# yinyunie/Pose2Room

Hardware: AMD Instinct MI355X
Metric: P2RNet train-step samples/sec (T=1024,J=53,bs=32) (higher is better)
Workload: dtype f32; 1 GPU; P2RNet full train step, bs=32/GPU, T=1024, J=53, seeds=512, proposals=128 (BASELINE configs[2]); input=P2RNet_dataloader over SyntheticPoseDataset, global_batch=32, frames=1024, parallelism=dp1

## Files before the change

### pose2room_amd/csrc/stgcn_gcn3_dcoef_body.h

```cpp
#include "gcn3_sched.inc"

#ifndef D3_MARK
#define D3_TRACE_TILE(tile)
#define D3_MARK(i)
#endif
namespace {

constexpr int D3_F = TILE_F, D3_NW = TILE_NW, D3_SLOTS = TILE_SLOTS, D3_V = TILE_V;
constexpr int D3_RS = TILE_RS, D3_BUF = TILE_BUF, D3_NV4 = TILE_NV4, D3_PW = TILE_PW;
static_assert(G3_V == TILE_V, "schedule generated for another skeleton");

struct D3Common {
  int T, ltot;
  int tiles_per_seq, total_tiles;
};
struct D3Params : D3Common, D3Extra {};

constexpr int d3_slot_joints[D3_NW][D3_SLOTS] = G3_SLOT_JOINTS_1;
constexpr int d3_plane0[D3_NW] = G3_PLANE0_1;

template <int NE, int O0, int O1, int O2, int O3, int O4, int O5>
__device__ __forceinline__ void d3_gather(const char *xl, float (&dv)[6][4]) {
  constexpr int off[6] = {O0, O1, O2, O3, O4, O5};
#pragma unroll
  for (int j = 0; j < NE; ++j)
#pragma unroll
    for (int q = 0; q < 4; ++q) dv[j][q] = *reinterpret_cast<const float *>(xl + off[j] + q * 4 * D3_RS * 4);
}

template <int CTRL>
__device__ __forceinline__ float d3_add_dpp(float v) {
  return v + __int_as_float(__builtin_amdgcn_update_dpp(0, __float_as_int(v), CTRL, 0xf, 0xf, true));
}
template <int OFF>
__device__ __forceinline__ void d3_lane_add(unsigned base, float v, unsigned long long mask) {
  asm volatile("s_mov_b64 exec, %2\n\tds_add_f32 %0, %1 offset:%3\n\ts_mov_b64 exec, -1"
               : : "v"(base), "v"(v), "s"(mask), "n"(OFF) : "memory");
}
template <int NE, int C0, int C1, int C2, int C3, int C4, int C5>
__device__ __forceinline__ void d3_reduce(const f32x4 &h, const float (&dv)[6][4], unsigned dcs) {
  constexpr unsigned long long L31 = 1ull << 31, L63 = 1ull << 63;
  constexpr int NP = NE / 2, NV = NP + (NE & 1);
  const f32x2 h01 = {h[0], h[1]}, h23 = {h[2], h[3]};
  float t[NE];
#pragma unroll
  for (int j = 0; j < NE; ++j) {
    f32x2 pr = h01 * f32x2{dv[j][0], dv[j][1]};
    pr = __builtin_elementwise_fma(h23, f32x2{dv[j][2], dv[j][3]}, pr);
    t[j] = pr.x + pr.y;
  }
  float v[NV];
#pragma unroll
  for (int q = 0; q < NP; ++q) {
    auto sw = __builtin_amdgcn_permlane32_swap(__float_as_uint(t[2 * q]), __float_as_uint(t[2 * q + 1]), false, false);
    v[q] = __uint_as_float(sw[0]) + __uint_as_float(sw[1]);
  }
  if (NE & 1) v[NP] = t[NE - 1];
#pragma unroll
  for (int q = 0; q < NV; ++q) v[q] = d3_add_dpp<0xB1>(v[q]);
#pragma unroll
  for (int q = 0; q < NV; ++q) v[q] = d3_add_dpp<0x4E>(v[q]);
#pragma unroll
  for (int q = 0; q < NV; ++q) v[q] = d3_add_dpp<0x141>(v[q]);
#pragma unroll
  for (int q = 0; q < NV; ++q) v[q] = d3_add_dpp<0x140>(v[q]);
#pragma unroll
  for (int q = 0; q < NV; ++q) v[q] = d3_add_dpp<0x142>(v[q]);
  if (NE & 1) v[NP] = d3_add_dpp<0x143>(v[NP]);
  if (NP > 0) { d3_lane_add<4 * C0>(dcs, v[0], L31); d3_lane_add<4 * C1>(dcs, v[0], L63); }
  if (NP > 1) { d3_lane_add<4 * C2>(dcs, v[1], L31); d3_lane_add<4 * C3>(dcs, v[1], L63); }
  if (NP > 2) { d3_lane_add<4 * C4>(dcs, v[2], L31); d3_lane_add<4 * C5>(dcs, v[2], L63); }
  if (NE == 1) d3_lane_add<4 * C0>(dcs, v[0], L63);
  if (NE == 3) d3_lane_add<4 * C2>(dcs, v[1], L63);
  if (NE == 5) d3_lane_add<4 * C4>(dcs, v[2], L63);
}

#define D3_VISIT(set, plane, next, wrap, piece)                                      \
  {                                                                                  \
    load_a(aS[(set) ^ 1], next, (wrap) ? ((ph + 1) & 3) : ph);                        \
    if ((piece) >= 0 && copy) dma_piece(piece);                                      \
  }
#define D3_STEP(set, slot, ne, o0, c0, o1, c1, o2, c2, o3, c3, o4, c4, o5, c5)   \
  {                                                                              \
    float dv_[6][4];                                                             \
    d3_gather<ne, o0, o1, o2, o3, o4, o5>(xl, dv_);                              \
    if (D3_FENCED) __builtin_amdgcn_sched_barrier(0);                            \
    d3_product(h, aS[set], bz[slot]);                                            \
    if (D3_FENCED) __builtin_amdgcn_sched_barrier(0);                            \
    d3_reduce<ne, c0, c1, c2, c3, c4, c5>(h, dv_, dcs_off);                      \
  }
#define D3_CONT(ne, o0, c0, o1, c1, o2, c2, o3, c3, o4, c4, o5, c5)   \
  {                                                                   \
    float dv_[6][4];                                                  \
    d3_gather<ne, o0, o1, o2, o3, o4, o5>(xl, dv_);                   \
    d3_reduce<ne, c0, c1, c2, c3, c4, c5>(h, dv_, dcs_off);           \
  }
#define D3_END(parity, pieces)                                                            \
  {                                                                                       \
    if (copy) { _Pragma("unroll") for (int i_ = pieces; i_ < D3_PW; ++i_) dma_piece(i_); } \
    if (parity) d3_copy_a(aS[0], aS[1]);                                                  \
  }

template <int WAVE>
__device__ __forceinline__ void d3_wave_main(const D3Params &p, float *lds, const float *__restrict__ x,
                                             const float *__restrict__ dz, const D3W *__restrict__ W, float xscale) {
  constexpr int V = D3_V, RS = D3_RS, BUF = D3_BUF, NW = D3_NW, SLOTS = D3_SLOTS;
  constexpr int wave = WAVE;
  unsigned dcs_off = (unsigned)(2 * BUF * sizeof(float));
  asm volatile("" : "+v"(dcs_off));
  const int tid = threadIdx.x;
  const int lane = tid & 63;
  const int g = lane >> 4, r = lane & 15;
  constexpr const int (&sj)[SLOTS] = d3_slot_joints[WAVE];

  const size_t row_stride = (size_t)p.T * V;
  const char *xl0 = reinterpret_cast<const char *>(lds + g * RS + r * V);

  int doff[D3_PW];
#pragma unroll
  for (int i = 0; i < D3_PW; ++i) {
    const int pc = i * NW + wave;
    const int e = pc * 64 + lane;
    const int lrow = e / (RS / 4), c4 = e - lrow * (RS / 4);
    const int row = 4 * (lrow & 3) + (lrow >> 2);
    doff[i] = (pc < TILE_PIECES && e < D3_NV4) ? (int)(((size_t)row * row_stride + 4 * c4) * sizeof(float)) : -1;
  }
  D3B bz[SLOTS];
  D3A aS[2];
  f32x4 h;
  auto load_a = [&](D3A &a, int k, int ph) { d3_load_a(a, W, k, ph, lane); };

  int tile = blockIdx.x;
  if (tile < p.total_tiles) {
    const int seq = tile / p.tiles_per_seq, t0 = (tile % p.tiles_per_seq) * D3_F;
    const float *dr = dz + (size_t)seq * 64 * row_stride + (size_t)t0 * V;
#pragma unroll
    for (int i = 0; i < D3_PW; ++i)
      if (doff[i] >= 0) tile_dma16(dr, doff[i], lds + (i * NW + wave) * 256);
  }
  load_a(aS[0], d3_plane0[WAVE], 0);

  for (; tile < p.total_tiles; tile += gridDim.x) {
    const int seq = tile / p.tiles_per_seq, t0 = (tile % p.tiles_per_seq) * D3_F;
    const float *dg = dz + (size_t)seq * 64 * row_stride + (size_t)t0 * V;
    const int ntile = tile + gridDim.x;
    const bool has_next = ntile < p.total_tiles;
    const int nseq = has_next ? ntile / p.tiles_per_seq : 0, nt0 = has_next ? (ntile % p.tiles_per_seq) * D3_F : 0;
    const float *ndg = dz + (size_t)nseq * 64 * row_stride + (size_t)nt0 * V;
    D3_TRACE_TILE(tile);
    D3_MARK(0);

    {
      float *xb = lds + BUF;
      const char *xr = reinterpret_cast<const char *>(xb + 4 * g * RS + r * V);
      const float *xs = x + (size_t)seq * 64 * row_stride + (size_t)t0 * V;
#pragma unroll
      for (int sl = 0; sl < 4; ++sl) {
        asm volatile("s_waitcnt lgkmcnt(0)" ::: "memory");
        __syncthreads();
#pragma unroll
        for (int i = 0; i < D3_PW; ++i)
          if (doff[i] >= 0) tile_dma16(xs + (size_t)sl * 16 * row_stride, doff[i], xb + (i * NW + wave) * 256);
        asm volatile("s_waitcnt vmcnt(0)" ::: "memory");
        __syncthreads();
#pragma unroll
        for (int i = 0; i < SLOTS; ++i)
          if (sj[i] >= 0) d3_read_x(bz[i], xr, sj[i], sl, xscale);
      }
      asm volatile("s_waitcnt lgkmcnt(0)" ::: "memory");
    }

#pragma unroll 1
    for (int ph = 0; ph < 4; ++ph) {
      D3_MARK(1 + 3 * ph);
      asm volatile("s_waitcnt vmcnt(0)" ::: "memory");
      D3_MARK(2 + 3 * ph);
      __syncthreads();
      D3_MARK(3 + 3 * ph);
      float *buf_nxt = lds + ((ph + 1) & 1) * BUF;
      const char *xl = xl0 + (ph & 1) * BUF * sizeof(float);
      const bool copy = ph + 1 < 4 || has_next;
      const float *src = (ph + 1 < 4) ? dg + (size_t)(ph + 1) * 16 * row_stride : ndg;
      auto dma_piece = [&](int i) {
        if (doff[i] >= 0) tile_dma16(src, doff[i], buf_nxt + (i * NW + wave) * 256);
      };
      if constexpr (WAVE == 0) { D3_BODY_0 } else if constexpr (WAVE == 1) { D3_BODY_1 }
      else if constexpr (WAVE == 2) { D3_BODY_2 } else if constexpr (WAVE == 3) { D3_BODY_3 }
      else if constexpr (WAVE == 4) { D3_BODY_4 } else if constexpr (WAVE == 5) { D3_BODY_5 }
      else if constexpr (WAVE == 6) { D3_BODY_6 } else { D3_BODY_7 }
    }
    D3_MARK(13);
  }
}

__global__ __launch_bounds__(D3_NW * 64, 2) void D3_KERNEL(D3Params p, const float *__restrict__ x,
                                                           const float *__restrict__ dz, const D3W *__restrict__ W,
                                                           float *__restrict__ dcoef_partial) {
  extern __shared__ float lds[];
  float *dcs = lds + 2 * D3_BUF;
  const int tid = threadIdx.x;
  for (int e = tid; e < p.ltot * D3_V; e += D3_NW * 64) dcs[e] = 0.f;
  float xscale, inv;
  d3_scales(p, xscale, inv);
  __syncthreads();
  switch (__builtin_amdgcn_readfirstlane(tid >> 6)) {
    case 0: d3_wave_main<0>(p, lds, x, dz, W, xscale); break;
    case 1: d3_wave_main<1>(p, lds, x, dz, W, xscale); break;
    case 2: d3_wave_main<2>(p, lds, x, dz, W, xscale); break;
    case 3: d3_wave_main<3>(p, lds, x, dz, W, xscale); break;
    case 4: d3_wave_main<4>(p, lds, x, dz, W, xscale); break;
    case 5: d3_wave_main<5>(p, lds, x, dz, W, xscale); break;
    case 6: d3_wave_main<6>(p, lds, x, dz, W, xscale); break;
    default: d3_wave_main<7>(p, lds, x, dz, W, xscale); break;
  }
  __syncthreads();
  float *out = dcoef_partial + (size_t)blockIdx.x * p.ltot * D3_V;
  for (int e = tid; e < p.ltot * D3_V; e += D3_NW * 64) out[e] = dcs[e] * inv;
}

int d3_launch(int N, int T, int V, int K, int ltot, const float *x, const float *dz, const D3W *W, int n_blocks,
              float *dcoef_partial, void *stream, const D3Extra &extra) {
  if (N < 0 || T <= 0 || V != D3_V || K != G3_K || ltot <= 0 || n_blocks < 1) return P2R_EINVAL;
  if (T % D3_F != 0 || ((uintptr_t)dz % 16) != 0) return P2R_EINVAL;
  if (N == 0) return hipMemsetAsync(dcoef_partial, 0, (size_t)n_blocks * ltot * V * sizeof(float), p2r_stream(stream));
  D3Params p;
  static_cast<D3Extra &>(p) = extra;
  p.T = T; p.ltot = ltot;
  p.tiles_per_seq = T / D3_F;
  const long long tiles = (long long)N * p.tiles_per_seq;
  if (tiles > 0x7fffffffLL) return P2R_EINVAL;
  p.total_tiles = (int)tiles;
  const size_t lds = (size_t)2 * D3_BUF * sizeof(float) + (size_t)ltot * V * sizeof(float);
  if (lds > 160 * 1024) return P2R_EINVAL;
  return p2r_launch_big_lds<D3_KERNEL>(n_blocks, D3_NW * 64, lds, stream, p, x, dz, W, dcoef_partial);
}

}
```

### pose2room_amd/csrc/stgcn_gcn3_dw.hip

```cpp
#include "stgcn_tile.h"

#include "gcn3_sched.inc"

namespace {

constexpr int W3_F = 4;
constexpr int W3_V = TILE_V;
constexpr int W3_NW = TILE_NW;
constexpr int W3_RL = W3_F * W3_V;
constexpr int W3_TILE = 64 * W3_RL;
constexpr int W3_NV4 = W3_TILE / 4;
constexpr int W3_PW = tile_pw(W3_NV4);
static_assert(G3_V == TILE_V, "schedule generated for another skeleton");
constexpr int W3_CS = (64 * W3_V + W3_NW * 64 - 1) / (W3_NW * 64);

struct W3Params {
  int T, ltot;
  int tiles_per_seq, total_tiles;
};

constexpr int w3_wave_set[W3_NW] = W3_WAVE_SET;
constexpr int w3_wave_half[W3_NW] = W3_WAVE_HALF;
constexpr int w3_set_planes[4][W3_MAXPL] = W3_SET_PLANES;

__device__ __forceinline__ void w3_mfma8(f32x4 (&acc)[2][4], const float (&a)[4], const f32x2 &b) {
  asm volatile(
      "s_nop 1\n\t"
      "v_mfma_f32_16x16x4_f32 %0, %8, %12, %0\n\tv_mfma_f32_16x16x4_f32 %1, %9, %12, %1\n\t"
      "v_mfma_f32_16x16x4_f32 %2, %10, %12, %2\n\tv_mfma_f32_16x16x4_f32 %3, %11, %12, %3\n\t"
      "v_mfma_f32_16x16x4_f32 %4, %8, %13, %4\n\tv_mfma_f32_16x16x4_f32 %5, %9, %13, %5\n\t"
      "v_mfma_f32_16x16x4_f32 %6, %10, %13, %6\n\tv_mfma_f32_16x16x4_f32 %7, %11, %13, %7"
      : "+v"(acc[0][0]), "+v"(acc[0][1]), "+v"(acc[0][2]), "+v"(acc[0][3]), "+v"(acc[1][0]), "+v"(acc[1][1]),
        "+v"(acc[1][2]), "+v"(acc[1][3])
      : "v"(a[0]), "v"(a[1]), "v"(a[2]), "v"(a[3]), "v"(b.x), "v"(b.y));
}

constexpr int W3_MAXNE = 12;

template <int NE>
__device__ __forceinline__ void w3_gather_n(const char *dl, const char *cl, const int (&off)[W3_MAXNE],
                                            const int (&ci)[W3_MAXNE], f32x2 (&dv)[W3_MAXNE], float (&cf)[W3_MAXNE]) {
#pragma unroll
  for (int j = 0; j < NE; ++j) {
    dv[j].x = *reinterpret_cast<const float *>(dl + off[j]);
    dv[j].y = *reinterpret_cast<const float *>(dl + off[j] + 16 * W3_RL * 4);
    cf[j] = *reinterpret_cast<const float *>(cl + 4 * ci[j]);
  }
}
template <int NE>
__device__ __forceinline__ f32x2 w3_combine(const f32x2 (&dv)[W3_MAXNE], const float (&cf)[W3_MAXNE]) {
  f32x2 v = dv[0] * f32x2{cf[0], cf[0]};
#pragma unroll
  for (int j = 1; j < NE; ++j) v = __builtin_elementwise_fma(dv[j], f32x2{cf[j], cf[j]}, v);
  return v;
}

#define W3_UNPACK(o0, c0, o1, c1, o2, c2, o3, c3, o4, c4, o5, c5, o6, c6, o7, c7, o8, c8, o9, c9, o10, c10, o11, c11) \
  constexpr int off_[W3_MAXNE] = {o0, o1, o2, o3, o4, o5, o6, o7, o8, o9, o10, o11};                                   \
  constexpr int ci_[W3_MAXNE] = {c0, c1, c2, c3, c4, c5, c6, c7, c8, c9, c10, c11};

#define W3_A(set, joint)                                                                            \
  {                                                                                                 \
    _Pragma("unroll") for (int m_ = 0; m_ < 4; ++m_)                                                \
        aS[set][m_] = *reinterpret_cast<const float *>(xl + 4 * (joint) + m_ * 16 * W3_RL * 4);      \
  }
#define W3_FIRST(ne, ...)                                        \
  {                                                              \
    W3_UNPACK(__VA_ARGS__)                                       \
    f32x2 dv_[W3_MAXNE]; float cf_[W3_MAXNE];                    \
    w3_gather_n<ne>(dl, cl, off_, ci_, dv_, cf_);                \
    b_cur = w3_combine<ne>(dv_, cf_);                            \
  }
#define W3_STEP(aset, slot, ne, ...)                             \
  {                                                              \
    W3_UNPACK(__VA_ARGS__)                                       \
    f32x2 dv_[W3_MAXNE]; float cf_[W3_MAXNE];                    \
    w3_gather_n<ne>(dl, cl, off_, ci_, dv_, cf_);                \
    __builtin_amdgcn_sched_barrier(0);                           \
    w3_mfma8(acc[slot], aS[aset], b_cur);                        \
    __builtin_amdgcn_sched_barrier(0);                           \
    b_cur = w3_combine<ne>(dv_, cf_);                            \
  }
#define W3_LAST(aset, slot)                \
  {                                        \
    __builtin_amdgcn_sched_barrier(0);     \
    w3_mfma8(acc[slot], aS[aset], b_cur);  \
  }

template <int WAVE>
__device__ __forceinline__ void w3_wave_main(const W3Params &p, float *lds, const float *__restrict__ x,
                                             const float *__restrict__ dz, float *__restrict__ dw_partial,
                                             float *__restrict__ colsum_partial) {
  constexpr int V = W3_V, RL = W3_RL, NW = W3_NW;
  constexpr int SET = w3_wave_set[WAVE], HALF = w3_wave_half[WAVE];
  constexpr int wave = WAVE;
  float *xs = lds;
  float *ds = lds + W3_TILE;
  float *coef_l = lds + 2 * W3_TILE;
  const int tid = threadIdx.x;
  const int lane = tid & 63;
  const int g = lane >> 4, r = lane & 15;
  const size_t row_stride = (size_t)p.T * V;

  const char *xl = reinterpret_cast<const char *>(xs + r * RL + g * V);
  const char *dl = reinterpret_cast<const char *>(ds + (32 * HALF + r) * RL + g * V);
  unsigned cl_off = (unsigned)((coef_l - lds) * sizeof(float));
  asm volatile("" : "+v"(cl_off));
  const char *cl = reinterpret_cast<const char *>(lds) + cl_off;

  unsigned doff[W3_PW];
#pragma unroll
  for (int i = 0; i < W3_PW; ++i) {
    const int pc = i * NW + wave, e = pc * 64 + lane;
    const int row = e / (RL / 4), c4 = e - row * (RL / 4);
    doff[i] = (pc < tile_pieces(W3_NV4) && e < W3_NV4) ? (unsigned)(((size_t)row * row_stride + 4 * c4) * sizeof(float)) : 0xffffffffu;
  }
  auto copy_tile = [&](int tile) {
    const int seq = tile / p.tiles_per_seq, t0 = (tile % p.tiles_per_seq) * W3_F;
    const float *xg = x + (size_t)seq * 64 * row_stride + (size_t)t0 * V;
    const float *dg = dz + (size_t)seq * 64 * row_stride + (size_t)t0 * V;
#pragma unroll
    for (int i = 0; i < W3_PW; ++i)
      if (doff[i] != 0xffffffffu) {
        tile_dma16(xg, doff[i], xs + (i * NW + wave) * 256);
        tile_dma16(dg, doff[i], ds + (i * NW + wave) * 256);
      }
  };

  f32x4 acc[W3_MAXPL][2][4];
#pragma unroll
  for (int s = 0; s < W3_MAXPL; ++s)
#pragma unroll
    for (int n = 0; n < 2; ++n)
#pragma unroll
      for (int m = 0; m < 4; ++m) acc[s][n][m] = f32x4{0.f, 0.f, 0.f, 0.f};
  float aS[2][4];
  f32x2 b_cur;
  float cs[W3_CS];
  int cso[W3_CS];
#pragma unroll
  for (int i = 0; i < W3_CS; ++i) {
    cs[i] = 0.f;
    const int idx = tid + NW * 64 * i;
    cso[i] = idx < 64 * V ? (idx / V) * RL + idx % V : 0;
  }

  const int per_xcd = (gridDim.x & 7) == 0 ? (int)(gridDim.x >> 3) : 0;
  const int xcd = blockIdx.x & 7, slot = blockIdx.x >> 3;
  auto tile_of = [&](int i) { return per_xcd ? (i * 8 + xcd) * per_xcd + slot : (int)(blockIdx.x + i * gridDim.x); };
  int it = 0;
  int tile = tile_of(0);
  for (int d = 0; d < (int)((per_xcd ? slot : blockIdx.x) & 3); ++d) __builtin_amdgcn_s_sleep(127);
  if (tile < p.total_tiles) copy_tile(tile);
  for (; tile < p.total_tiles; tile = tile_of(++it)) {
    asm volatile("s_waitcnt vmcnt(0)" ::: "memory");
    __syncthreads();

    if (colsum_partial) {
      float dv4[W3_CS][4];
#pragma unroll
      for (int i = 0; i < W3_CS; ++i)
#pragma unroll
        for (int f = 0; f < 4; ++f) dv4[i][f] = ds[cso[i] + f * V];
#pragma unroll
      for (int i = 0; i < W3_CS; ++i) cs[i] += (dv4[i][0] + dv4[i][1]) + (dv4[i][2] + dv4[i][3]);
    }
    if constexpr (SET == 0) { W3_BODY_0 } else if constexpr (SET == 1) { W3_BODY_1 }
    else if constexpr (SET == 2) { W3_BODY_2 } else { W3_BODY_3 }

    __syncthreads();
    const int ntile = tile_of(it + 1);
    if (ntile < p.total_tiles) copy_tile(ntile);
  }

  if (colsum_partial) {
#pragma unroll
    for (int i = 0; i < W3_CS; ++i) {
      const int idx = tid + NW * 64 * i;
      if (idx < 64 * V) colsum_partial[(size_t)blockIdx.x * 64 * V + idx] = cs[i];
    }
  }
  float *out = dw_partial + (size_t)blockIdx.x * G3_K * 64 * 64;
#pragma unroll
  for (int s = 0; s < W3_MAXPL; ++s) {
    const int k = w3_set_planes[SET][s];
    if (k < 0) continue;
#pragma unroll
    for (int n = 0; n < 2; ++n)
#pragma unroll
      for (int m = 0; m < 4; ++m)
#pragma unroll
        for (int q = 0; q < 4; ++q)
          out[((size_t)k * 64 + 16 * m + 4 * g + q) * 64 + 32 * HALF + 16 * n + r] = acc[s][n][m][q];
  }
}

__global__ __launch_bounds__(W3_NW * 64, 2) void gcn3_dw_kernel(W3Params p, const float *__restrict__ x,
                                                                const float *__restrict__ dz,
                                                                const float *__restrict__ coef,
                                                                float *__restrict__ dw_partial,
                                                                float *__restrict__ colsum_partial) {
  extern __shared__ float lds[];
  float *coef_l = lds + 2 * W3_TILE;
  const int tid = threadIdx.x;
  for (int e = tid; e < p.ltot * W3_V; e += W3_NW * 64) coef_l[e] = coef[e];
  __syncthreads();
  switch (__builtin_amdgcn_readfirstlane(tid >> 6)) {
    case 0: w3_wave_main<0>(p, lds, x, dz, dw_partial, colsum_partial); break;
    case 1: w3_wave_main<1>(p, lds, x, dz, dw_partial, colsum_partial); break;
    case 2: w3_wave_main<2>(p, lds, x, dz, dw_partial, colsum_partial); break;
    case 3: w3_wave_main<3>(p, lds, x, dz, dw_partial, colsum_partial); break;
    case 4: w3_wave_main<4>(p, lds, x, dz, dw_partial, colsum_partial); break;
    case 5: w3_wave_main<5>(p, lds, x, dz, dw_partial, colsum_partial); break;
    case 6: w3_wave_main<6>(p, lds, x, dz, dw_partial, colsum_partial); break;
    default: w3_wave_main<7>(p, lds, x, dz, dw_partial, colsum_partial); break;
  }
}

}

extern "C" int p2r_stgcn_gcn3_weight_grad(int N, int T, int V, int K, int ltot, const float *x, const float *dz,
                                          const float *coef, int n_blocks, float *dw_partial, float *colsum_partial,
                                          void *stream) {
  if (N < 0 || T <= 0 || V != W3_V || K != G3_K || ltot <= 0 || n_blocks < 1) return P2R_EINVAL;
  if (T % W3_F != 0 || T > (1 << 20) || ((uintptr_t)x % 16) != 0 || ((uintptr_t)dz % 16) != 0) return P2R_EINVAL;
  if (N == 0) {
    hipError_t e = hipMemsetAsync(dw_partial, 0, (size_t)n_blocks * K * 64 * 64 * sizeof(float), p2r_stream(stream));
    if (e == hipSuccess && colsum_partial)
      e = hipMemsetAsync(colsum_partial, 0, (size_t)n_blocks * 64 * V * sizeof(float), p2r_stream(stream));
    return (int)e;
  }
  W3Params p;
  p.T = T; p.ltot = ltot;
  p.tiles_per_seq = T / W3_F;
  const long long tiles = (long long)N * p.tiles_per_seq;
  if (tiles > 0x7fffffffLL) return P2R_EINVAL;
  p.total_tiles = (int)tiles;
  const size_t lds = (size_t)2 * W3_TILE * sizeof(float) + (size_t)ltot * V * sizeof(float);
  if (lds > 160 * 1024) return P2R_EINVAL;
  return p2r_launch_big_lds<gcn3_dw_kernel>(n_blocks, W3_NW * 64, lds, stream, p, x, dz, coef, dw_partial, colsum_partial);
}
```

### pose2room_amd/csrc/stgcn_gcn3_grad.hip

```cpp
#include "stgcn_tile.h"

#ifdef P2R_CYCLE_TRACE
__device__ unsigned long long d3_trace[8 * 32];
#define D3_TRACE_TILE(tile) const bool trace_on = blockIdx.x == 7 && (tile) == 7 + 3 * (int)gridDim.x
#define D3_MARK(i) do { if (trace_on && lane == 0) d3_trace[wave * 32 + (i)] = __builtin_readcyclecounter(); } while (0)
#endif
#define D3_KERNEL gcn3_dcoef_kernel
namespace {

typedef float D3A[16];
typedef float D3B[16];
typedef float D3W;
struct D3Extra {};
constexpr bool D3_FENCED = true;
__device__ __forceinline__ void d3_scales(const D3Extra &, float &xscale, float &inv) { xscale = 1.f; inv = 1.f; }
__device__ __forceinline__ void d3_copy_a(D3A &dst, const D3A &src) {
#pragma unroll
  for (int e = 0; e < 16; ++e) dst[e] = src[e];
}

__device__ __forceinline__ void d3_product(f32x4 &h, const D3A &a, const D3B &b) {
  asm volatile(
      "s_nop 1\n\t"
      "v_mfma_f32_16x16x4_f32 %0, %1, %9, 0\n\tv_mfma_f32_16x16x4_f32 %0, %2, %10, %0\n\t"
      "v_mfma_f32_16x16x4_f32 %0, %3, %11, %0\n\tv_mfma_f32_16x16x4_f32 %0, %4, %12, %0\n\t"
      "v_mfma_f32_16x16x4_f32 %0, %5, %13, %0\n\tv_mfma_f32_16x16x4_f32 %0, %6, %14, %0\n\t"
      "v_mfma_f32_16x16x4_f32 %0, %7, %15, %0\n\tv_mfma_f32_16x16x4_f32 %0, %8, %16, %0"
      : "=&v"(h)
      : "v"(a[0]), "v"(a[1]), "v"(a[2]), "v"(a[3]), "v"(a[4]), "v"(a[5]), "v"(a[6]), "v"(a[7]),
        "v"(b[0]), "v"(b[1]), "v"(b[2]), "v"(b[3]), "v"(b[4]), "v"(b[5]), "v"(b[6]), "v"(b[7]));
  asm volatile(
      "v_mfma_f32_16x16x4_f32 %0, %1, %9, %0\n\tv_mfma_f32_16x16x4_f32 %0, %2, %10, %0\n\t"
      "v_mfma_f32_16x16x4_f32 %0, %3, %11, %0\n\tv_mfma_f32_16x16x4_f32 %0, %4, %12, %0\n\t"
      "v_mfma_f32_16x16x4_f32 %0, %5, %13, %0\n\tv_mfma_f32_16x16x4_f32 %0, %6, %14, %0\n\t"
      "v_mfma_f32_16x16x4_f32 %0, %7, %15, %0"
      : "+v"(h)
      : "v"(a[8]), "v"(a[9]), "v"(a[10]), "v"(a[11]), "v"(a[12]), "v"(a[13]), "v"(a[14]), "v"(a[15]),
        "v"(b[8]), "v"(b[9]), "v"(b[10]), "v"(b[11]), "v"(b[12]), "v"(b[13]), "v"(b[14]), "v"(b[15]));
  h = __builtin_amdgcn_mfma_f32_16x16x4f32(a[15], b[15], h, 0, 0, 0);
}

__device__ __forceinline__ void d3_load_a(D3A &a, const float *__restrict__ Wp, int k, int ph, int lane) {
#pragma unroll
  for (int pp = 0; pp < 4; ++pp) {
    const float4 u = reinterpret_cast<const float4 *>(Wp)[((size_t)(k * 4 + pp) * 4 + ph) * 64 + lane];
    a[4 * pp + 0] = u.x; a[4 * pp + 1] = u.y; a[4 * pp + 2] = u.z; a[4 * pp + 3] = u.w;
  }
}
__device__ __forceinline__ void d3_read_x(D3B &b, const char *xr, int joint, int sl, float) {
#pragma unroll
  for (int kp = 0; kp < 4; ++kp) b[4 * sl + kp] = *reinterpret_cast<const float *>(xr + (kp * TILE_RS + joint) * 4);
}

}
#include "stgcn_gcn3_dcoef_body.h"

#ifdef P2R_CYCLE_TRACE
extern "C" int p2r_debug_d3_trace(unsigned long long *dst) {
  return (int)hipMemcpyFromSymbol(dst, HIP_SYMBOL(d3_trace), sizeof(d3_trace));
}
#endif

extern "C" int p2r_stgcn_gcn3_coef_grad(int N, int T, int V, int K, int ltot, const float *x, const float *dz,
                                        const float *Wp, int n_blocks, float *dcoef_partial, void *stream) {
  if (T > (1 << 20) || ((uintptr_t)x % 4) != 0) return P2R_EINVAL;
  return d3_launch(N, T, V, K, ltot, x, dz, Wp, n_blocks, dcoef_partial, stream, D3Extra{});
}
```

### pose2room_amd/csrc/stgcn_gcn3h_grad.hip

```cpp
#include "stgcn_tile.h"
#include "split16.h"

#pragma clang diagnostic ignored "-Warray-bounds"

#define D3_KERNEL gcn3h_dcoef_kernel
namespace {

struct D3A { p2r_h8 p[2], q[2]; };
struct D3B { p2r_h8 p[2], q[2]; };
typedef p2r_h8 D3W;
struct D3Extra {
  const unsigned *x_amax;
  const float *winv;
};
#ifdef D3_NO_FENCE
constexpr bool D3_FENCED = false;
#else
constexpr bool D3_FENCED = true;
#endif
__device__ __forceinline__ void d3_scales(const D3Extra &e, float &xscale, float &inv) {
  float xinv;
  p2r_split_scale(e.x_amax, xscale, xinv);
  inv = xinv * e.winv[0];
}
__device__ __forceinline__ void d3_copy_a(D3A &dst, const D3A &src) { dst = src; }

__device__ __forceinline__ void d3_product(f32x4 &h, const D3A &a, const D3B &b) {
  f32x4 acc = {0.f, 0.f, 0.f, 0.f};
#pragma unroll
  for (int ks = 0; ks < 2; ++ks) {
    acc = __builtin_amdgcn_mfma_f32_16x16x32_f16(a.p[ks], b.q[ks], acc, 0, 0, 0);
    acc = __builtin_amdgcn_mfma_f32_16x16x32_f16(a.q[ks], b.p[ks], acc, 0, 0, 0);
  }
#pragma unroll
  for (int ks = 0; ks < 2; ++ks) acc = __builtin_amdgcn_mfma_f32_16x16x32_f16(a.p[ks], b.p[ks], acc, 0, 0, 0);
  h = acc;
}

__device__ __forceinline__ void d3_load_a(D3A &a, const p2r_h8 *__restrict__ Wd, int k, int ph, int lane) {
  const p2r_h8 *wd = Wd + ((size_t)(k * 4 + ph) * 2 * 2) * 64 + lane;
  a.p[0] = wd[0]; a.p[1] = wd[64]; a.q[0] = wd[128]; a.q[1] = wd[192];
}
__device__ __forceinline__ void d3_read_x(D3B &b, const char *xr, int joint, int sl, float xscale) {
  float v4[4];
#pragma unroll
  for (int kp = 0; kp < 4; ++kp) v4[kp] = *reinterpret_cast<const float *>(xr + (kp * TILE_RS + joint) * 4) * xscale;
#pragma unroll
  for (int kp = 0; kp < 4; kp += 2) {
    p2r_f2 xx = {v4[kp], v4[kp + 1]};
    asm volatile("" : "+v"(xx));
    const p2r_h2 ph_ = __builtin_convertvector(xx, p2r_h2);
    const p2r_h2 qh_ = __builtin_convertvector(xx - __builtin_convertvector(ph_, p2r_f2), p2r_h2);
    b.p[sl >> 1][4 * (sl & 1) + kp] = ph_.x; b.p[sl >> 1][4 * (sl & 1) + kp + 1] = ph_.y;
    b.q[sl >> 1][4 * (sl & 1) + kp] = qh_.x; b.q[sl >> 1][4 * (sl & 1) + kp + 1] = qh_.y;
  }
}

}
#include "stgcn_gcn3_dcoef_body.h"

extern "C" int p2r_stgcn_gcn3h_coef_grad(int N, int T, int V, int K, int ltot, const float *x, const float *dz,
                                         const void *Wd, const float *winv, int n_blocks, float *dcoef_partial,
                                         const unsigned *x_amax, void *stream) {
  if (!Wd || !winv || T > (1 << 19) || ((uintptr_t)x % 16) != 0 || ((uintptr_t)Wd % 16) != 0) return P2R_EINVAL;
  if (n_blocks > 65535) return P2R_EINVAL;
  return d3_launch(N, T, V, K, ltot, x, dz, reinterpret_cast<const p2r_h8 *>(Wd), n_blocks, dcoef_partial, stream,
                   D3Extra{x_amax, winv});
}
```

Baseline: 799.5 samples/s.

## Hand-schedule LDS gathers and packed FMAs into reserved VGPRs in GCN3 grad kernels

Replaces the compiler-generated LDS gathers and packed multiply/FMA reductions in the dcoef and dw backward kernels with inline assembly. The assembly writes into a fixed block of high VGPRs that are kept out of the allocator by capping it with amdgpu_num_vgpr. LDS addresses become plain 32-bit offsets, and the weight-fragment loads switch to raw buffer loads with immediate offsets. The aim is to cut address arithmetic and register pressure and to control instruction placement around the MFMAs. In exchange, correctness now depends on hand-tuned s_nop hazard padding and hardcoded register numbers.

```diff
diff --git a/pose2room_amd/csrc/stgcn_gcn3_dcoef_body.h b/pose2room_amd/csrc/stgcn_gcn3_dcoef_body.h
--- a/pose2room_amd/csrc/stgcn_gcn3_dcoef_body.h
+++ b/pose2room_amd/csrc/stgcn_gcn3_dcoef_body.h
@@ -19,13 +19,54 @@
 constexpr int d3_slot_joints[D3_NW][D3_SLOTS] = G3_SLOT_JOINTS_1;
 constexpr int d3_plane0[D3_NW] = G3_PLANE0_1;
 
-template <int NE, int O0, int O1, int O2, int O3, int O4, int O5>
-__device__ __forceinline__ void d3_gather(const char *xl, float (&dv)[6][4]) {
-  constexpr int off[6] = {O0, O1, O2, O3, O4, O5};
-#pragma unroll
-  for (int j = 0; j < NE; ++j)
-#pragma unroll
-    for (int q = 0; q < 4; ++q) dv[j][q] = *reinterpret_cast<const float *>(xl + off[j] + q * 4 * D3_RS * 4);
+constexpr int D3_QS = 4 * D3_RS * 4;
+#define D3_RD(J, R0, R1, R2, R3)                                                                             \
+  if constexpr ((J) < ne_)                                                                                   \
+    asm volatile("ds_read_b32 " R0 ", %0 offset:%1\n\tds_read_b32 " R1 ", %0 offset:%2\n\t"                  \
+                 "ds_read_b32 " R2 ", %0 offset:%3\n\tds_read_b32 " R3 ", %0 offset:%4"                      \
+                 : : "v"(xl), "n"(off_[J]), "n"(off_[J] + D3_QS), "n"(off_[J] + 2 * D3_QS), "n"(off_[J] + 3 * D3_QS) \
+                 : "memory", R0, R1, R2, R3);
+#define D3_GATHER(ne, o0, o1, o2, o3, o4, o5)                                              \
+  constexpr int off_[6] = {o0, o1, o2, o3, o4, o5};                                        \
+  constexpr int ne_ = ne;                                                                  \
+  D3_RD(0, "v184", "v185", "v186", "v187") D3_RD(1, "v188", "v189", "v190", "v191")        \
+  D3_RD(2, "v192", "v193", "v194", "v195") D3_RD(3, "v196", "v197", "v198", "v199")        \
+  D3_RD(4, "v200", "v201", "v202", "v203") D3_RD(5, "v204", "v205", "v206", "v207")
+
+#define D3_PM(J, D) "v_pk_mul_f32 %[p" #J "], %[h01], " D "\n\t"
+#define D3_PF(J, D) "v_pk_fma_f32 %[p" #J "], %[h23], " D ", %[p" #J "]\n\t"
+#define D3_PK1 D3_PM(0, "v[184:185]") "s_nop 0\n\t" D3_PF(0, "v[186:187]")
+#define D3_PK2 D3_PM(0, "v[184:185]") D3_PM(1, "v[188:189]") D3_PF(0, "v[186:187]") D3_PF(1, "v[190:191]")
+#define D3_PK3 D3_PM(0, "v[184:185]") D3_PM(1, "v[188:189]") D3_PM(2, "v[192:193]") \
+               D3_PF(0, "v[186:187]") D3_PF(1, "v[190:191]") D3_PF(2, "v[194:195]")
+#define D3_PK4 D3_PM(0, "v[184:185]") D3_PM(1, "v[188:189]") D3_PM(2, "v[192:193]") D3_PM(3, "v[196:197]") \
+               D3_PF(0, "v[186:187]") D3_PF(1, "v[190:191]") D3_PF(2, "v[194:195]") D3_PF(3, "v[198:199]")
+#define D3_PK5 D3_PM(0, "v[184:185]") D3_PM(1, "v[188:189]") D3_PM(2, "v[192:193]") D3_PM(3, "v[196:197]") \
+               D3_PM(4, "v[200:201]") D3_PF(0, "v[186:187]") D3_PF(1, "v[190:191]") D3_PF(2, "v[194:195]") \
+               D3_PF(3, "v[198:199]") D3_PF(4, "v[202:203]")
+#define D3_PK6 D3_PM(0, "v[184:185]") D3_PM(1, "v[188:189]") D3_PM(2, "v[192:193]") D3_PM(3, "v[196:197]") \
+               D3_PM(4, "v[200:201]") D3_PM(5, "v[204:205]") D3_PF(0, "v[186:187]") D3_PF(1, "v[190:191]") \
+               D3_PF(2, "v[194:195]") D3_PF(3, "v[198:199]") D3_PF(4, "v[202:203]") D3_PF(5, "v[206:207]")
+#define D3_PO1 [p0] "=&v"(pr[0])
+#define D3_PO2 D3_PO1, [p1] "=&v"(pr[1])
+#define D3_PO3 D3_PO2, [p2] "=&v"(pr[2])
+#define D3_PO4 D3_PO3, [p3] "=&v"(pr[3])
+#define D3_PO5 D3_PO4, [p4] "=&v"(pr[4])
+#define D3_PO6 D3_PO5, [p5] "=&v"(pr[5])
+#define D3_PROD(N)                                                                                              \
+  {                                                                                                             \
+    if constexpr (FRESH)                                                                                        \
+      asm volatile("s_waitcnt lgkmcnt(0)\n\t" D3_H_READY "\n\t" D3_PK##N "s_nop 0"                              \
+                   : D3_PO##N : [h01] "v"(h01), [h23] "v"(h23) : "memory");                                     \
+    else                                                                                                        \
+      asm volatile("s_waitcnt lgkmcnt(0)\n\t" D3_PK##N "s_nop 0" : D3_PO##N : [h01] "v"(h01), [h23] "v"(h23) : "memory"); \
+  }
+template <int NE, bool FRESH>
+__device__ __forceinline__ void d3_products(const f32x4 &h, f32x2 (&pr)[6]) {
+  static_assert(NE >= 1 && NE <= 6, "entries per step");
+  const f32x2 h01 = {h[0], h[1]}, h23 = {h[2], h[3]};
+  if constexpr (NE == 1) D3_PROD(1) else if constexpr (NE == 2) D3_PROD(2) else if constexpr (NE == 3) D3_PROD(3)
+  else if constexpr (NE == 4) D3_PROD(4) else if constexpr (NE == 5) D3_PROD(5) else D3_PROD(6)
 }
 
 template <int CTRL>
@@ -37,18 +78,15 @@
   asm volatile("s_mov_b64 exec, %2\n\tds_add_f32 %0, %1 offset:%3\n\ts_mov_b64 exec, -1"
                : : "v"(base), "v"(v), "s"(mask), "n"(OFF) : "memory");
 }
-template <int NE, int C0, int C1, int C2, int C3, int C4, int C5>
-__device__ __forceinline__ void d3_reduce(const f32x4 &h, const float (&dv)[6][4], unsigned dcs) {
+template <int NE, bool FRESH, int C0, int C1, int C2, int C3, int C4, int C5>
+__device__ __forceinline__ void d3_reduce(const f32x4 &h, unsigned dcs) {
   constexpr unsigned long long L31 = 1ull << 31, L63 = 1ull << 63;
   constexpr int NP = NE / 2, NV = NP + (NE & 1);
-  const f32x2 h01 = {h[0], h[1]}, h23 = {h[2], h[3]};
+  f32x2 pr[6];
+  d3_products<NE, FRESH>(h, pr);
   float t[NE];
 #pragma unroll
-  for (int j = 0; j < NE; ++j) {
-    f32x2 pr = h01 * f32x2{dv[j][0], dv[j][1]};
-    pr = __builtin_elementwise_fma(h23, f32x2{dv[j][2], dv[j][3]}, pr);
-    t[j] = pr.x + pr.y;
-  }
+  for (int j = 0; j < NE; ++j) t[j] = pr[j].x + pr[j].y;
   float v[NV];
 #pragma unroll
   for (int q = 0; q < NP; ++q) {
@@ -82,18 +120,16 @@
   }
 #define D3_STEP(set, slot, ne, o0, c0, o1, c1, o2, c2, o3, c3, o4, c4, o5, c5)   \
   {                                                                              \
-    float dv_[6][4];                                                             \
-    d3_gather<ne, o0, o1, o2, o3, o4, o5>(xl, dv_);                              \
+    D3_GATHER(ne, o0, o1, o2, o3, o4, o5)                                        \
     if (D3_FENCED) __builtin_amdgcn_sched_barrier(0);                            \
     d3_product(h, aS[set], bz[slot]);                                            \
     if (D3_FENCED) __builtin_amdgcn_sched_barrier(0);                            \
-    d3_reduce<ne, c0, c1, c2, c3, c4, c5>(h, dv_, dcs_off);                      \
+    d3_reduce<ne, true, c0, c1, c2, c3, c4, c5>(h, dcs_off);                     \
   }
 #define D3_CONT(ne, o0, c0, o1, c1, o2, c2, o3, c3, o4, c4, o5, c5)   \
   {                                                                   \
-    float dv_[6][4];                                                  \
-    d3_gather<ne, o0, o1, o2, o3, o4, o5>(xl, dv_);                   \
-    d3_reduce<ne, c0, c1, c2, c3, c4, c5>(h, dv_, dcs_off);           \
+    D3_GATHER(ne, o0, o1, o2, o3, o4, o5)                             \
+    d3_reduce<ne, false, c0, c1, c2, c3, c4, c5>(h, dcs_off);         \
   }
 #define D3_END(parity, pieces)                                                            \
   {                                                                                       \
@@ -114,7 +150,7 @@
   constexpr const int (&sj)[SLOTS] = d3_slot_joints[WAVE];
 
   const size_t row_stride = (size_t)p.T * V;
-  const char *xl0 = reinterpret_cast<const char *>(lds + g * RS + r * V);
+  const unsigned xl0 = (unsigned)((g * RS + r * V) * sizeof(float));
 
   int doff[D3_PW];
 #pragma unroll
@@ -178,7 +214,7 @@
       __syncthreads();
       D3_MARK(3 + 3 * ph);
       float *buf_nxt = lds + ((ph + 1) & 1) * BUF;
-      const char *xl = xl0 + (ph & 1) * BUF * sizeof(float);
+      const unsigned xl = xl0 + (unsigned)((ph & 1) * BUF * sizeof(float));
       const bool copy = ph + 1 < 4 || has_next;
       const float *src = (ph + 1 < 4) ? dg + (size_t)(ph + 1) * 16 * row_stride : ndg;
       auto dma_piece = [&](int i) {
@@ -193,9 +229,9 @@
   }
 }
 
-__global__ __launch_bounds__(D3_NW * 64, 2) void D3_KERNEL(D3Params p, const float *__restrict__ x,
-                                                           const float *__restrict__ dz, const D3W *__restrict__ W,
-                                                           float *__restrict__ dcoef_partial) {
+__global__ __launch_bounds__(D3_NW * 64, 2) __attribute__((amdgpu_num_vgpr(184))) void D3_KERNEL(
+    D3Params p, const float *__restrict__ x, const float *__restrict__ dz, const D3W *__restrict__ W,
+    float *__restrict__ dcoef_partial) {
   extern __shared__ float lds[];
   float *dcs = lds + 2 * D3_BUF;
   const int tid = threadIdx.x;
diff --git a/pose2room_amd/csrc/stgcn_gcn3_dw.hip b/pose2room_amd/csrc/stgcn_gcn3_dw.hip
--- a/pose2room_amd/csrc/stgcn_gcn3_dw.hip
+++ b/pose2room_amd/csrc/stgcn_gcn3_dw.hip
@@ -36,22 +36,48 @@
 }
 
 constexpr int W3_MAXNE = 12;
-
+constexpr int W3_NROW = 16 * W3_RL * 4;
+
+#define W3_RD(J, X, Y, C)                                                                                         \
+  if constexpr ((J) < ne_)                                                                                        \
+    asm volatile("ds_read_b32 " X ", %0 offset:%2\n\tds_read_b32 " Y ", %0 offset:%3\n\tds_read_b32 " C ", %1 offset:%4" \
+                 : : "v"(dl), "v"(cl), "n"(off_[J]), "n"(off_[J] + W3_NROW), "n"(4 * ci_[J]) : "memory", X, Y, C);
+#define W3_GATHER                                                                                   \
+  W3_RD(0, "v204", "v205", "v192") W3_RD(1, "v206", "v207", "v193") W3_RD(2, "v208", "v209", "v194")   \
+  W3_RD(3, "v210", "v211", "v195") W3_RD(4, "v212", "v213", "v196") W3_RD(5, "v214", "v215", "v197")   \
+  W3_RD(6, "v216", "v217", "v198") W3_RD(7, "v218", "v219", "v199") W3_RD(8, "v220", "v221", "v200")   \
+  W3_RD(9, "v222", "v223", "v201") W3_RD(10, "v224", "v225", "v202") W3_RD(11, "v226", "v227", "v203")
+
+#define W3_CE(D, C) "s_nop 0\n\tv_pk_fma_f32 %0, " D ", " C ", %0 op_sel_hi:[1,0,1]\n\t"
+#define W3_CO(D, C) "s_nop 0\n\tv_pk_fma_f32 %0, " D ", " C ", %0 op_sel:[0,1,0] op_sel_hi:[1,1,1]\n\t"
+#define W3_C1 "s_waitcnt lgkmcnt(0)\n\tv_pk_mul_f32 %0, v[204:205], v[192:193] op_sel_hi:[1,0]\n\t"
+#define W3_C2 W3_C1 W3_CO("v[206:207]", "v[192:193]")
+#define W3_C3 W3_C2 W3_CE("v[208:209]", "v[194:195]")
+#define W3_C4 W3_C3 W3_CO("v[210:211]", "v[194:195]")
+#define W3_C5 W3_C4 W3_CE("v[212:213]", "v[196:197]")
+#define W3_C6 W3_C5 W3_CO("v[214:215]", "v[196:197]")
+#define W3_C7 W3_C6 W3_CE("v[216:217]", "v[198:199]")
+#define W3_C8 W3_C7 W3_CO("v[218:219]", "v[198:199]")
+#define W3_C9 W3_C8 W3_CE("v[220:221]", "v[200:201]")
+#define W3_C10 W3_C9 W3_CO("v[222:223]", "v[200:201]")
+#define W3_C11 W3_C10 W3_CE("v[224:225]", "v[202:203]")
+#define W3_C12 W3_C11 W3_CO("v[226:227]", "v[202:203]")
 template <int NE>
-__device__ __forceinline__ void w3_gather_n(const char *dl, const char *cl, const int (&off)[W3_MAXNE],
-                                            const int (&ci)[W3_MAXNE], f32x2 (&dv)[W3_MAXNE], float (&cf)[W3_MAXNE]) {
-#pragma unroll
-  for (int j = 0; j < NE; ++j) {
-    dv[j].x = *reinterpret_cast<const float *>(dl + off[j]);
-    dv[j].y = *reinterpret_cast<const float *>(dl + off[j] + 16 * W3_RL * 4);
-    cf[j] = *reinterpret_cast<const float *>(cl + 4 * ci[j]);
-  }
-}
-template <int NE>
-__device__ __forceinline__ f32x2 w3_combine(const f32x2 (&dv)[W3_MAXNE], const float (&cf)[W3_MAXNE]) {
-  f32x2 v = dv[0] * f32x2{cf[0], cf[0]};
-#pragma unroll
-  for (int j = 1; j < NE; ++j) v = __builtin_elementwise_fma(dv[j], f32x2{cf[j], cf[j]}, v);
+__device__ __forceinline__ f32x2 w3_combine() {
+  static_assert(NE >= 1 && NE <= W3_MAXNE, "entries per unit");
+  f32x2 v;
+  if constexpr (NE == 1) asm volatile(W3_C1 "s_nop 0" : "=v"(v) : : "memory");
+  else if constexpr (NE == 2) asm volatile(W3_C2 "s_nop 0" : "=v"(v) : : "memory");
+  else if constexpr (NE == 3) asm volatile(W3_C3 "s_nop 0" : "=v"(v) : : "memory");
+  else if constexpr (NE == 4) asm volatile(W3_C4 "s_nop 0" : "=v"(v) : : "memory");
+  else if constexpr (NE == 5) asm volatile(W3_C5 "s_nop 0" : "=v"(v) : : "memory");
+  else if constexpr (NE == 6) asm volatile(W3_C6 "s_nop 0" : "=v"(v) : : "memory");
+  else if constexpr (NE == 7) asm volatile(W3_C7 "s_nop 0" : "=v"(v) : : "memory");
+  else if constexpr (NE == 8) asm volatile(W3_C8 "s_nop 0" : "=v"(v) : : "memory");
+  else if constexpr (NE == 9) asm volatile(W3_C9 "s_nop 0" : "=v"(v) : : "memory");
+  else if constexpr (NE == 10) asm volatile(W3_C10 "s_nop 0" : "=v"(v) : : "memory");
+  else if constexpr (NE == 11) asm volatile(W3_C11 "s_nop 0" : "=v"(v) : : "memory");
+  else asm volatile(W3_C12 "s_nop 0" : "=v"(v) : : "memory");
   return v;
 }
 
@@ -59,27 +85,29 @@
   constexpr int off_[W3_MAXNE] = {o0, o1, o2, o3, o4, o5, o6, o7, o8, o9, o10, o11};                                   \
   constexpr int ci_[W3_MAXNE] = {c0, c1, c2, c3, c4, c5, c6, c7, c8, c9, c10, c11};
 
-#define W3_A(set, joint)                                                                            \
-  {                                                                                                 \
-    _Pragma("unroll") for (int m_ = 0; m_ < 4; ++m_)                                                \
-        aS[set][m_] = *reinterpret_cast<const float *>(xl + 4 * (joint) + m_ * 16 * W3_RL * 4);      \
-  }
+#define W3_A(set, joint)                                                                                          \
+  asm volatile("ds_read_b32 %0, %4 offset:%5\n\tds_read_b32 %1, %4 offset:%6\n\t"                                  \
+               "ds_read_b32 %2, %4 offset:%7\n\tds_read_b32 %3, %4 offset:%8"                                      \
+               : "=&v"(aS[set][0]), "=&v"(aS[set][1]), "=&v"(aS[set][2]), "=&v"(aS[set][3])                        \
+               : "v"(xl), "n"(4 * (joint)), "n"(4 * (joint) + W3_NROW), "n"(4 * (joint) + 2 * W3_NROW),            \
+                 "n"(4 * (joint) + 3 * W3_NROW)                                                                    \
+               : "memory");
 #define W3_FIRST(ne, ...)                                        \
   {                                                              \
     W3_UNPACK(__VA_ARGS__)                                       \
-    f32x2 dv_[W3_MAXNE]; float cf_[W3_MAXNE];                    \
-    w3_gather_n<ne>(dl, cl, off_, ci_, dv_, cf_);                \
-    b_cur = w3_combine<ne>(dv_, cf_);                            \
+    constexpr int ne_ = ne;                                      \
+    W3_GATHER                                                    \
+    b_cur = w3_combine<ne>();                                    \
   }
 #define W3_STEP(aset, slot, ne, ...)                             \
   {                                                              \
     W3_UNPACK(__VA_ARGS__)                                       \
-    f32x2 dv_[W3_MAXNE]; float cf_[W3_MAXNE];                    \
-    w3_gather_n<ne>(dl, cl, off_, ci_, dv_, cf_);                \
+    constexpr int ne_ = ne;                                      \
+    W3_GATHER                                                    \
     __builtin_amdgcn_sched_barrier(0);                           \
     w3_mfma8(acc[slot], aS[aset], b_cur);                        \
     __builtin_amdgcn_sched_barrier(0);                           \
-    b_cur = w3_combine<ne>(dv_, cf_);                            \
+    b_cur = w3_combine<ne>();                                    \
   }
 #define W3_LAST(aset, slot)                \
   {                                        \
@@ -96,17 +124,14 @@
   constexpr int wave = WAVE;
   float *xs = lds;
   float *ds = lds + W3_TILE;
-  float *coef_l = lds + 2 * W3_TILE;
   const int tid = threadIdx.x;
   const int lane = tid & 63;
   const int g = lane >> 4, r = lane & 15;
   const size_t row_stride = (size_t)p.T * V;
 
-  const char *xl = reinterpret_cast<const char *>(xs + r * RL + g * V);
-  const char *dl = reinterpret_cast<const char *>(ds + (32 * HALF + r) * RL + g * V);
-  unsigned cl_off = (unsigned)((coef_l - lds) * sizeof(float));
-  asm volatile("" : "+v"(cl_off));
-  const char *cl = reinterpret_cast<const char *>(lds) + cl_off;
+  const unsigned xl = (unsigned)((r * RL + g * V) * sizeof(float));
+  const unsigned dl = (unsigned)((W3_TILE + (32 * HALF + r) * RL + g * V) * sizeof(float));
+  const unsigned cl = (unsigned)(2 * W3_TILE * sizeof(float));
 
   unsigned doff[W3_PW];
 #pragma unroll
@@ -195,11 +220,9 @@
   }
 }
 
-__global__ __launch_bounds__(W3_NW * 64, 2) void gcn3_dw_kernel(W3Params p, const float *__restrict__ x,
-                                                                const float *__restrict__ dz,
-                                                                const float *__restrict__ coef,
-                                                                float *__restrict__ dw_partial,
-                                                                float *__restrict__ colsum_partial) {
+__global__ __launch_bounds__(W3_NW * 64, 2) __attribute__((amdgpu_num_vgpr(192))) void gcn3_dw_kernel(
+    W3Params p, const float *__restrict__ x, const float *__restrict__ dz, const float *__restrict__ coef,
+    float *__restrict__ dw_partial, float *__restrict__ colsum_partial) {
   extern __shared__ float lds[];
   float *coef_l = lds + 2 * W3_TILE;
   const int tid = threadIdx.x;
diff --git a/pose2room_amd/csrc/stgcn_gcn3_grad.hip b/pose2room_amd/csrc/stgcn_gcn3_grad.hip
--- a/pose2room_amd/csrc/stgcn_gcn3_grad.hip
+++ b/pose2room_amd/csrc/stgcn_gcn3_grad.hip
@@ -5,6 +5,7 @@
 #define D3_TRACE_TILE(tile) const bool trace_on = blockIdx.x == 7 && (tile) == 7 + 3 * (int)gridDim.x
 #define D3_MARK(i) do { if (trace_on && lane == 0) d3_trace[wave * 32 + (i)] = __builtin_readcyclecounter(); } while (0)
 #endif
+#define D3_H_READY "s_nop 9"
 #define D3_KERNEL gcn3_dcoef_kernel
 namespace {
 
@@ -41,10 +42,13 @@
 }
 
 __device__ __forceinline__ void d3_load_a(D3A &a, const float *__restrict__ Wp, int k, int ph, int lane) {
+  const auto rs = __builtin_amdgcn_make_buffer_rsrc(const_cast<float *>(Wp), (short)0, 0x7fffffff, 0x00027000);
+  const unsigned vo = (unsigned)lane * 16u;
 #pragma unroll
   for (int pp = 0; pp < 4; ++pp) {
-    const float4 u = reinterpret_cast<const float4 *>(Wp)[((size_t)(k * 4 + pp) * 4 + ph) * 64 + lane];
-    a[4 * pp + 0] = u.x; a[4 * pp + 1] = u.y; a[4 * pp + 2] = u.z; a[4 * pp + 3] = u.w;
+    const auto u = __builtin_amdgcn_raw_buffer_load_b128(rs, vo, ((k * 4 + pp) * 4 + ph) * 1024, 0);
+    a[4 * pp + 0] = __uint_as_float(u[0]); a[4 * pp + 1] = __uint_as_float(u[1]);
+    a[4 * pp + 2] = __uint_as_float(u[2]); a[4 * pp + 3] = __uint_as_float(u[3]);
   }
 }
 __device__ __forceinline__ void d3_read_x(D3B &b, const char *xr, int joint, int sl, float) {
diff --git a/pose2room_amd/csrc/stgcn_gcn3h_grad.hip b/pose2room_amd/csrc/stgcn_gcn3h_grad.hip
--- a/pose2room_amd/csrc/stgcn_gcn3h_grad.hip
+++ b/pose2room_amd/csrc/stgcn_gcn3h_grad.hip
@@ -3,6 +3,7 @@
 
 #pragma clang diagnostic ignored "-Warray-bounds"
 
+#define D3_H_READY "s_nop 7"
 #define D3_KERNEL gcn3h_dcoef_kernel
 namespace {
 
@@ -38,8 +39,13 @@
 }
 
 __device__ __forceinline__ void d3_load_a(D3A &a, const p2r_h8 *__restrict__ Wd, int k, int ph, int lane) {
-  const p2r_h8 *wd = Wd + ((size_t)(k * 4 + ph) * 2 * 2) * 64 + lane;
-  a.p[0] = wd[0]; a.p[1] = wd[64]; a.q[0] = wd[128]; a.q[1] = wd[192];
+  const auto rs = __builtin_amdgcn_make_buffer_rsrc(const_cast<p2r_h8 *>(Wd), (short)0, 0x7fffffff, 0x00027000);
+  const unsigned vo = (unsigned)lane * 16u;
+  p2r_h8 u[4];
+#pragma unroll
+  for (int i = 0; i < 4; ++i)
+    u[i] = __builtin_bit_cast(p2r_h8, __builtin_amdgcn_raw_buffer_load_b128(rs, vo, ((k * 4 + ph) * 4 + i) * 1024, 0));
+  a.p[0] = u[0]; a.p[1] = u[1]; a.q[0] = u[2]; a.q[1] = u[3];
 }
 __device__ __forceinline__ void d3_read_x(D3B &b, const char *xr, int joint, int sl, float xscale) {
   float v4[4];
```

Result: no change. 802.5 samples/s, median of 6 (+0.4%).
